# Keyteer/Mixed-precision_LU_Factorization

Hardware: AMD Instinct MI355X
Metric: LU GFLOP/s at N=32768 (1/2/4/8 GPUs); IR iterations to ||r||/||b||<1e-12 (higher is better)
Workload: dtype f64

## Files before the change

include/mpf_c.h:

```cpp
#ifndef MPF_C_H
#define MPF_C_H
#include <stdint.h>
#ifdef __cplusplus
extern "C" {
#endif

typedef struct mpf_ctx mpf_ctx;

enum { MPF_TRAIL_FP64 = 0, MPF_TRAIL_FP16 = 1, MPF_TRAIL_FP16X3 = 2 };

typedef struct mpf_opts {
    int32_t trailing;
    int32_t verbose;
    int32_t fused_panel;
    int32_t sync_timing;
    int32_t no_lookahead;
    int32_t superpanel;
    int32_t pivot_path;
    int32_t pivot_search;
} mpf_opts;

typedef struct mpf_stats {
    double ms_total;
    double ms_h2d, ms_d2h;
// ... 3 lines not shown
    int32_t hpanel_timeouts;
    int32_t info;
    int32_t gemm_launches;
    int32_t lookahead;
    int32_t superpanel;
    int32_t pivot_path;
    double gemm_flops;
    double gemm_bytes;
    double ms_gemm_big, gemm_big_flops, gemm_big_bytes;
    double ms_cvt;
    double ms_blockrow;
    int32_t gemm_big_launches;
    int32_t host_rows_streamed;
    int32_t host_late_segments;
    int32_t pivot_search;
} mpf_stats;

int mpf_create(mpf_ctx **out, int device);
int mpf_destroy(mpf_ctx *ctx);
int mpf_set_stream(mpf_ctx *ctx, void *hip_stream);
int mpf_synchronize(mpf_ctx *ctx);
const char *mpf_last_error(mpf_ctx *ctx);
int mpf_get_stats(mpf_ctx *ctx, mpf_stats *out);
int64_t mpf_hgetf2_capacity_rows(mpf_ctx *ctx, int32_t waiters, int32_t form);
int mpf_set_option(mpf_ctx *ctx, const char *name, int64_t value);
int mpf_get_option(mpf_ctx *ctx, const char *name, int64_t *value);
int mpf_option_name(int32_t index, char *buf, int64_t buflen);
int mpf_device_report(char *buf, int64_t buflen);


// ... 200 lines not shown
```

mixed-precision_lu_factorization_amd/__init__.py:

```python
import ctypes as C
import os
import subprocess

_HERE = os.path.dirname(os.path.abspath(__file__))
LIB_PATH = os.environ.get("MPF_LIB") or os.path.join(_HERE, "lib", "libmpf_amd.so")
PROBE_LIB_PATH = os.environ.get("MPF_PROBE_LIB") or os.path.join(_HERE, "lib", "libmpf_probe.so")

TRAIL_FP64 = 0
TRAIL_FP16 = 1
TRAIL_FP16X3 = 2

C_ABI_SYMBOLS = [
    "mpf_create", "mpf_destroy", "mpf_set_stream", "mpf_synchronize", "mpf_last_error", "mpf_get_stats",
    "mpf_device_report", "mpf_factor_host", "mpf_factor_dev", "mpf_double_to_fp16", "mpf_hdiv",
    "mpf_hgetf2_pivots", "mpf_hgetf2", "mpf_laswp", "mpf_dgetf2_npv", "mpf_dtrsm_llnu", "mpf_dgemm_minus",
    "mpf_solve_ir", "mpf_hgetf2_capacity_rows", "mpf_set_option", "mpf_get_option", "mpf_option_name", "mpf_hgemm_minus", "mpf_hgemm_minus_f32", "mpf_w32_from_f64", "mpf_w32_to_f64", "mpf_w32_laswp", "mpf_gesv", "mpf_matgen_dev", "mpf_matgen_cols_dev",
    "mpf_matgen_state", "mpf_rccl_unique_id", "mpf_rccl_init", "mpf_rccl_destroy", "mpf_rccl_version", "mpf_rccl_info", "mpf_rccl_bcast_probe", "mpf_factor_dist",
    "mpf_solve_ir_dist", "mpf_rccl_selftest", "mpf_check_plu_dev", "mpf_check_plu_host", "mpf_solve_ir_nrhs",
    "mpf_solve_gmres_ir", "mpf_trim", "mpf_dist_set_p2p",
    "mpf_solve_ir_trans", "mpf_lange", "mpf_geequ", "mpf_gecon", "mpf_gesvx",
    "mpf_getrs", "mpf_solve_ir_block", "mpf_gerfs", "mpf_gesvx_block",
    "mpf_dgetf2_piv", "mpf_solve_gmres_ir_block", "mpf_dgetf2_tp",
    "mpf_residual_x", "mpf_gerfsx",
]
# ... 3 lines not shown

class MpfOpts(C.Structure):
    _fields_ = [("trailing", C.c_int32), ("verbose", C.c_int32), ("fused_panel", C.c_int32),
                ("sync_timing", C.c_int32), ("no_lookahead", C.c_int32), ("superpanel", C.c_int32), ("pivot_path", C.c_int32), ("pivot_search", C.c_int32)]


class MpfStats(C.Structure):
    _fields_ = [("ms_total", C.c_double), ("ms_h2d", C.c_double), ("ms_d2h", C.c_double),
                ("ms_hpanel", C.c_double), ("ms_laswp", C.c_double), ("ms_dpanel", C.c_double),
                ("ms_trsm", C.c_double), ("ms_gemm", C.c_double), ("n", C.c_int64), ("nb", C.c_int32),
                ("panels", C.c_int32), ("hpanel_timeouts", C.c_int32), ("info", C.c_int32),
                ("gemm_launches", C.c_int32), ("lookahead", C.c_int32), ("superpanel", C.c_int32),
                ("pivot_path", C.c_int32), ("gemm_flops", C.c_double), ("gemm_bytes", C.c_double),
                ("ms_gemm_big", C.c_double), ("gemm_big_flops", C.c_double), ("gemm_big_bytes", C.c_double),
                ("ms_cvt", C.c_double), ("ms_blockrow", C.c_double), ("gemm_big_launches", C.c_int32), ("host_rows_streamed", C.c_int32),
                ("host_late_segments", C.c_int32), ("pivot_search", C.c_int32)]


class MpfIrStats(C.Structure):
    _fields_ = [("iterations", C.c_int32), ("converged", C.c_int32), ("rel_residual", C.c_double),
                ("history", C.c_double * 32), ("ms_total", C.c_double), ("stalled", C.c_int32), ("reserved", C.c_int32)]


class MpfGmresStats(C.Structure):
    _fields_ = [("outer_iterations", C.c_int32), ("inner_iterations", C.c_int32), ("converged", C.c_int32), ("budget_expired", C.c_int32),
                ("rel_residual", C.c_double), ("history", C.c_double * 32), ("ms_total", C.c_double)]


class MpfRcclInfo(C.Structure):
    _fields_ = [("version", C.c_int32), ("has_comm", C.c_int32), ("comm_count", C.c_int32), ("comm_rank", C.c_int32), ("has_p2p", C.c_int32),
                ("device", C.c_int32), ("visible_devices", C.c_int32), ("reserved", C.c_int32),
# ... 728 lines not shown
```

mixed-precision_lu_factorization_amd/csrc/laswp.hip:

```cpp
#include "mpf_internal.h"

constexpr int LASWP_CPB = 16;

__global__ __launch_bounds__(256) void laswp_plan_kernel(const int *ipiv, int k, int cols, MovedList *out) {
    __shared__ int slot[HP_MAXCOLS];
    __shared__ int rowof[2 * HP_MAXCOLS];
    __shared__ int content[2 * HP_MAXCOLS];
    __shared__ int used[2 * HP_MAXCOLS];
    __shared__ int count;
    const int t = threadIdx.x;
    for (int s = t; s < 2 * cols; s += 256) { content[s] = s; used[s] = s < cols; rowof[s] = s < cols ? k + s : -1; }
    if (t == 0) count = 0;
    __syncthreads();
    if (t < cols) {
        const int p = ipiv[t] - 1;
        int s;
        if (p < k + cols) s = p - k;
        else {
            int first = t;
            for (int i = 0; i < t; ++i)
                if (ipiv[i] - 1 == p) { first = i; break; }
            s = cols + first;
            if (first == t) { rowof[s] = p; used[s] = 1; }
        }
// ... 376 lines not shown
        const int64_t rows = N - r0;
        if (rows <= 0) continue;
        for (int b = p - sb; b < p; ++b) {
            if (world > 1 && b % world != rank) continue;
            const int w = nb;
            dim3 grid((unsigned)((rows + 255) / 256), (unsigned)((w + 15) / 16));
            double *Ab = A + (int64_t)(world > 1 ? b / world : b) * nb * lda;
            if (gather) lazy_gather_kernel<<<grid, 256, 0, c->stream>>>(Ab, lda, N, r0, w, Gmap, c->perm_tmp, rows);
            else lazy_scatter_kernel<<<grid, 256, 0, c->stream>>>(Ab, lda, N, r0, w, c->Fmap, c->perm_tmp, rows);
            lazy_copyback_kernel<<<grid, 256, 0, c->stream>>>(Ab, lda, N, r0, w, c->perm_tmp, rows);
        }
    }
    MPF_HIP_TRY(c, hipGetLastError());
    return 0;
}
```

mixed-precision_lu_factorization_amd/csrc/mpf_host.cpp:

```cpp
#include "solve_common.h"
#include "../../include/MPF.h"
#include <climits>
#include <cstdio>
#include <cstdlib>
#include <cstring>
#include <cmath>
#include <iostream>
#include <vector>
#include <mutex>
#include <functional>
#include <chrono>

static thread_local std::string g_noctx_err;

namespace {
struct OptDesc { const char *name, *env; size_t off; bool wide; long long lo, hi; };
#define OPT_I(field, env, lo, hi) {#field, env, offsetof(MpfTuning, field), false, lo, hi}
#define OPT_L(field, env, lo, hi) {#field, env, offsetof(MpfTuning, field), true, lo, hi}
const OptDesc kOpts[] = {
    OPT_I(safe_pivots, "MPF_SAFE_PIVOTS", 0, 1),
    OPT_I(pivot_fp64, "MPF_PIVOT_FP64", 0, 2),
    OPT_I(chain_pipeline, "MPF_CHAIN_PIPELINE", 0, 1),
    OPT_L(chain_pipeline_below, "MPF_CHAIN_PIPELINE_BELOW", 0, 1ll << 40),
    OPT_I(fp16_work32, "MPF_FP16_WORK32", 0, 1),
// ... 1 lines not shown
    OPT_I(superpanel_fp64, "MPF_SUPERPANEL_FP64", 1, 8),
    OPT_I(no_lookahead, "MPF_NO_LOOKAHEAD", 0, 1),
    OPT_I(verbose, "MPF_VERBOSE", 0, 1),
    OPT_I(timeline, "MPF_TIMELINE", 0, 1),
    OPT_L(hp_spin_limit, "MPF_HP_SPIN_LIMIT", 1, 1ll << 31),
    OPT_L(hp_gate_ticks, "MPF_HP_GATE_TICKS", 0, 1ll << 40),
    OPT_I(hp_acq_fence, "MPF_HP_ACQ_FENCE", 0, 1),
    OPT_I(hp_window, "MPF_HP_WINDOW", -1, 1 << 30),
    OPT_I(hgemm_pad, "MPF_HGEMM_PAD", 0, 65536),
    OPT_I(hgemm_split_pad, "MPF_HGEMM_SPLIT_PAD", 0, 65536),
    OPT_I(hgemm_big, "MPF_HGEMM_BIG", 0, 1),
    OPT_I(hgemm_big_tile, "MPF_HGEMM_BIG_TILE", 0, 5),
    OPT_I(hgemm_mfma16, "MPF_HGEMM_MFMA16", 0, 1),
    OPT_I(dgemm_dma, "MPF_DGEMM_DMA", 0, 1),
    OPT_I(lazy_gather, "MPF_LAZY_GATHER", 0, 1),
    OPT_I(dpanel_fused_form, "MPF_DPANEL_FUSED", 0, 1),
    OPT_I(dist_instalments, "MPF_DIST_INSTALMENTS", 0, 1),
    OPT_L(dist_instalment_min_bytes, "MPF_DIST_INSTALMENT_MIN_BYTES", 0, 1ll << 40),
    OPT_I(generic_fused, "MPF_GENERIC_FUSED", 0, 1),
    OPT_I(fp64_rowmajor, "MPF_FP64_ROWMAJOR", 0, 1),
    OPT_L(fp64_rowmajor_min_n, "MPF_FP64_ROWMAJOR_MIN_N", 0, 1ll << 40),
    OPT_I(trsm_laswp_fused, "MPF_TRSM_LASWP_FUSED", 0, 1),
    OPT_I(fp64_two_lanes, "MPF_FP64_TWO_LANES", 0, 1 << 30),
    OPT_I(fp64_lane_a_pct, "MPF_FP64_LANE_A_PCT", 20, 90),
    OPT_I(fp64_pair, "MPF_FP64_PAIR", 0, 1),
    OPT_L(fp64_pair_min_n, "MPF_FP64_PAIR_MIN_N", 0, 1ll << 40),
    OPT_I(event_timers, "MPF_EVENT_TIMERS", 0, 2),
    OPT_I(dist_world1_loop, "MPF_DIST_WORLD1_LOOP", 0, 1),
    OPT_I(gesv_fp64_tflops, "MPF_GESV_FP64_TFLOPS", 0, 1000),
    OPT_I(gate_wait_value, "MPF_GATE_WAIT_VALUE", 0, 1),
// ... 51 lines not shown
    if (e != hipSuccess || ndev == 0) return fail(nullptr, -3, "No HIP devices available.");
    if (device < 0 || device >= ndev) return fail(nullptr, -1, "mpf_create: bad device index");
    mpf_ctx *c = new mpf_ctx();
    tuning_from_env(c->tune);
    c->device = device;
    if (hipSetDevice(device) != hipSuccess) { delete c; return fail(nullptr, -2, "hipSetDevice failed"); }
    hipDeviceProp_t prop;
    if (hipGetDeviceProperties(&prop, device) == hipSuccess) c->num_cus = prop.multiProcessorCount;
    if (hipStreamCreateWithFlags(&c->stream, hipStreamNonBlocking) != hipSuccess) { delete c; return fail(nullptr, -2, "hipStreamCreate failed"); }
    c->own_stream = true;
    {
        int lo = 0, hi = 0;
        hipDeviceGetStreamPriorityRange(&lo, &hi);
        if (hipStreamCreateWithPriority(&c->pstream, hipStreamNonBlocking, hi) != hipSuccess) c->pstream = nullptr;
        if (hipStreamCreateWithPriority(&c->tstream, hipStreamNonBlocking, hi) != hipSuccess) c->tstream = nullptr;
    }
    if (hipMalloc((void **)&c->ws, sizeof(MpfWorkspace)) != hipSuccess) { hipStreamDestroy(c->stream); delete c; return fail(nullptr, -2, "hipMalloc(workspace) failed"); }
    hipMemset(c->ws, 0, sizeof(MpfWorkspace));
    if (hipExtMallocWithFlags((void **)&c->hp_signal, 8, hipMallocSignalMemory) != hipSuccess) { c->hp_signal = nullptr; (void)hipGetLastError(); }
    else hipMemset(c->hp_signal, 0, 8);
    hipEventCreate(&c->ev0);
    hipEventCreate(&c->ev1);
    *out = c;
    return 0;
}

int mpf_destroy(mpf_ctx *c) {
    if (!c) return 0;
    hipSetDevice(c->device);
    if (c->stream) hipStreamSynchronize(c->stream);
    if (c->ws) hipFree(c->ws);
    if (c->hp_signal) hipFree(c->hp_signal);
    mpf_rccl_destroy(c);
    sink_destroy(c);
    feed_destroy(c);
    if (c->ev0) hipEventDestroy(c->ev0);
    if (c->ev1) hipEventDestroy(c->ev1);
    if (c->pstream) { hipStreamSynchronize(c->pstream); hipStreamDestroy(c->pstream); }
    if (c->tstream) { hipStreamSynchronize(c->tstream); hipStreamDestroy(c->tstream); }
    if (c->xstream) { hipStreamSynchronize(c->xstream); hipStreamDestroy(c->xstream); }
    for (hipEvent_t e : c->ev_pool) hipEventDestroy(e);
    if (c->own_stream && c->stream) hipStreamDestroy(c->stream);
    delete c;
    return 0;
}

int mpf_set_stream(mpf_ctx *c, void *hip_stream) {
    if (!c) return -1;
    if (c->own_stream && c->stream) { hipStreamSynchronize(c->stream); hipStreamDestroy(c->stream); }
    c->stream = (hipStream_t)hip_stream;
    c->own_stream = false;
    return 0;
}

// ... 406 lines not shown
        StreamSwap sw(c, T);
        r.rc = ev.timed(f.st.ms_dpanel, T, [&] {
            int e = 0;
            for (int s = 0; s < np && !e; ++s) {
                e = launch_laswp_block_gated(c, f.d_A + nx * lda, lda, pc2, (int)nx + 32 * s, 32, f.d_ipiv + nx + 32 * s, N, 32 * (s + 1));
                if (!e) e = launch_dgetf2_npv_piece(c, Anx, lda, (int)(N - nx), pc2, f.o.fused_panel, (int)nx, s);
            }
            return e; });
        r.b = ev.get();
        hipEventRecord(r.b, T);
    }
    f.st.panels++;
    return r;
}

static int factor_epilogue(const FactorArgs &f, int rc, bool sink, int sb, bool side_streams) {
    mpf_ctx *c = f.c;
    hipStream_t S = c->stream;
    const int npanels = (int)((f.N + f.nb - 1) / f.nb);
    if (sink) sink_notify(c, npanels, S);
    else if (!rc) rc = f.ev.timed(f.st.ms_laswp, S, [&] { return launch_lazy_left_swaps(c, f.d_A, f.lda, f.N, f.nb, npanels, c->lists, sb); });
    hipError_t se = sink_stream_wait(c, S);
    hipError_t sp = side_streams ? sink_stream_wait(c, c->pstream) : hipSuccess;
    if (side_streams && c->tstream) { const hipError_t stt = sink_stream_wait(c, c->tstream); if (sp == hipSuccess) sp = stt; }
    if (!rc && (se != hipSuccess || sp != hipSuccess))
        return fail(c, -2, std::string("factorization failed: ") + hipGetErrorString(se != hipSuccess ? se : sp));
    f.ev.collect();
    f.st.lookahead = side_streams ? 1 : 0;
    return rc;
}

static int factor_lookahead(mpf_ctx *c, double *d_A, int64_t lda, int64_t N, int32_t nb, int32_t *d_ipiv,
                            const mpf_opts &o, mpf_stats &st) {
    hipStream_t S = c->stream, P = c->pstream;
    EvPool ev(c);
    ev.keep = &st.ms_gemm;
// ... 63 lines not shown
    return factor_epilogue(f, rc, sink, 1, true);
}

static bool pivots_fit_beside_update(const mpf_ctx *c, int64_t rows) {
    return c->num_cus <= 0 || (rows + HP_R - 1) / HP_R <= (int64_t)c->num_cus * 4 / 5;
}

static bool lane_split(const mpf_ctx *c, int64_t lo, int64_t hi, int64_t &cm) {
    const int64_t cw = hi - lo;
    if (cm >= 0 && (cm - lo) * 100 >= cw * (c->tune.fp64_lane_a_pct - 10)) return false;
    cm = lo + ((cw * c->tune.fp64_lane_a_pct / 100 + 127) / 128) * 128;
    if (cm > hi - 128) cm = hi - 128;
    return true;
}

struct PairHandover {
    int64_t k0 = 0;
    hipEvent_t chain = nullptr;
    hipEvent_t doneL = nullptr, doneR = nullptr;
    int64_t cm = -1;
};

static int factor_rm_pairs(mpf_ctx *c, EvPool &ev, mpf_stats &st, const mpf_opts &o, double *d_A, int64_t lda, int64_t N, int32_t nb,
                           int32_t *d_ipiv, hipEvent_t init_done, PairHandover &h) {
    hipStream_t S = c->stream, P = c->pstream, T = c->tstream;
    double *R = c->r64;
    const int64_t ldr = N, ldp = 2 * (int64_t)nb;
    const FactorArgs f{c, ev, st, o, d_A, lda, N, nb, d_ipiv};
    int rc = 0;
    hipEvent_t doneX = nullptr, doneA = nullptr, doneB = nullptr;
    int64_t cm = -1;
    int64_t k = h.k0;
    struct { bool valid = false; int64_t k = 0, c_lo = 0, w = 0; double *PI2 = nullptr; hipEvent_t ready = nullptr; } pendB;
    auto far_update = [&](int64_t kk, double *pi2, int64_t c_lo, int64_t w) -> int {
        const int64_t r0 = kk + 2 * (int64_t)nb;
        const int e = ev.timed(st.ms_gemm, S, [&] { return launch_dgemm_minus(c, w, N - r0, 2 * nb, R + kk * ldr + c_lo, ldr, pi2, ldp, R + r0 * ldr + c_lo, ldr); });
        count_gemm(st, o, N - r0, w, 2 * nb);
        return e;
    };
// ... 6 lines not shown
        hipEventRecord(doneB, S);
        pendB.valid = false;
        return e;
    };
    for (; rc == 0; k += 2 * (int64_t)nb) {
        const int64_t k1 = k + nb, k2 = k1 + nb, k3 = k2 + nb, k5 = k3 + 2 * (int64_t)nb;
        if (k5 + 256 > N || (N - k1) <= c->tune.fp64_pair_min_n) break;
        if (!pivots_fit_beside_update(c, N - k1)) break;
        const bool resplit = lane_split(c, k5, N, cm);
        double *Ak = d_A + k * lda + k, *Ak1 = d_A + k1 * lda + k1;
        double *PI = c->rm_pair + ((k / (2 * nb)) & 1) * N * ldp;
        double *PI2 = PI + (int64_t)nb * ldp;
        const MovedList *lk = c->lists + (k / nb), *lk1 = c->lists + (k1 / nb);
        hipEvent_t lt_ready = ev.get(), e1 = ev.get(), inner_done = ev.get(), chain1 = ev.get(), pi_ready = ev.get(), e2 = ev.get(),
                   chain2 = ev.get(), evX = ev.get(), evA = ev.get(), evB = ev.get(), ps1 = ev.get(), ps2 = ev.get();
        {
            if (doneB) hipStreamWaitEvent(P, doneB, 0);
            StreamSwap sw(c, P);
            rc = ev.timed(st.ms_cvt, P, [&] { return launch_transpose64(c, Ak + nb, lda, PI, ldp, N - k1, nb, true); });
            hipEventRecord(lt_ready, P);
        }
        if (rc) break;
        {
            hipStreamWaitEvent(T, h.chain, 0);
            hipStreamWaitEvent(T, doneX ? doneX : init_done, 0);
            StreamSwap sw(c, T);
            rc = ev.timed(st.ms_laswp, T, [&] { return launch_laswp_from_list_rm64(c, R + k1, ldr, k3 - k1, lk, (int64_t)LASWP_MAXMOVED * k1); });
            if (!rc) rc = ev.timed(st.ms_trsm, T, [&] { return launch_dtrsm_llnu_strided(c, nb, nb, Ak, lda, R + k * ldr + k1, ldr, 1); });
            hipStreamWaitEvent(T, lt_ready, 0);
            if (!rc) rc = ev.timed(st.ms_gemm, T, [&] { return launch_dgemm_minus(c, nb, N - k1, nb, R + k * ldr + k1, ldr, PI, ldp, R + k1 * ldr + k1, ldr); });
// ... 1 lines not shown
            if (!rc) rc = ev.timed(st.ms_cvt, T, [&] { return launch_transpose64(c, Ak1, lda, R + k1 * ldr + k1, ldr, N - k1, nb, false); });
            hipEventRecord(e1, T);
            if (!rc) rc = ev.timed(st.ms_trsm, T, [&] { return launch_dtrsm_llnu_strided(c, nb, nb, Ak, lda, R + k * ldr + k2, ldr, 1); });
            if (!rc) rc = ev.timed(st.ms_gemm, T, [&] { return launch_dgemm_minus(c, nb, N - k1, nb, R + k * ldr + k2, ldr, PI, ldp, R + k1 * ldr + k2, ldr); });
            count_gemm(st, o, N - k1, nb, nb);
            if (!rc) rc = ev.timed(st.ms_cvt, T, [&] { return launch_transpose64(c, d_A + k1 * lda + k, lda, R + k * ldr + k1, ldr, nb, k3 - k1, false); });
            hipEventRecord(inner_done, T);
        }
        if (rc) break;
        {
            hipStreamWaitEvent(P, e1, 0);
            if (doneA) hipStreamWaitEvent(P, doneA, 0);
            hipEventRecord(ps1, P);
            rc = panel_chain(f, k1, P);
            hipEventRecord(chain1, P);
            StreamSwap sw(c, P);
            hipStreamWaitEvent(P, inner_done, 0);
            if (!rc) rc = ev.timed(st.ms_laswp, P, [&] { return launch_laswp_from_list_rm64(c, PI - k1 * ldp, ldp, nb, lk1, 0); });
            if (!rc) rc = ev.timed(st.ms_cvt, P, [&] { return launch_transpose64(c, Ak1 + nb, lda, PI2 + nb, ldp, N - k2, nb, true); });
            hipEventRecord(pi_ready, P);
        }
        if (!rc) rc = flush_B(ps1);
        if (rc) break;
        {
            hipStreamWaitEvent(T, chain1, 0);
            StreamSwap sw(c, T);
            rc = ev.timed(st.ms_laswp, T, [&] { return launch_laswp_from_list_rm64(c, R + k2, ldr, nb, lk1, (int64_t)LASWP_MAXMOVED * k2); });
            if (!rc) rc = ev.timed(st.ms_trsm, T, [&] { return launch_dtrsm_llnu_strided(c, nb, nb, Ak1, lda, R + k1 * ldr + k2, ldr, 1); });
            hipStreamWaitEvent(T, pi_ready, 0);
            if (!rc) rc = ev.timed(st.ms_gemm, T, [&] { return launch_dgemm_minus(c, nb, N - k2, nb, R + k1 * ldr + k2, ldr, PI2 + nb, ldp, R + k2 * ldr + k2, ldr); });
// ... 45 lines not shown
        if (rc) break;
        doneA = ev.get();
        hipEventRecord(doneA, S);
        {
            if (doneB) hipStreamWaitEvent(T, doneB, 0);
            StreamSwap sw(c, T);
            rc = far_prep(cm, N - cm);
            hipEventRecord(evB, T);
        }
        if (rc) break;
        pendB.valid = true; pendB.k = k; pendB.PI2 = PI2; pendB.c_lo = cm; pendB.w = N - cm; pendB.ready = evB;
        h.chain = chain2;
        if (o.verbose) printf("panels k=%lld, %lld rows=%lld (row-major copy, paired: far update K = %d, lanes split at %lld)\n", (long long)k1, (long long)k2, (long long)(N - k1), 2 * nb, (long long)cm);
    }
    if (!rc) rc = flush_B(nullptr);
    h.k0 = k;
    h.doneL = doneA; h.doneR = doneB; h.cm = cm;
    return rc;
}

static int factor_lookahead_rm(mpf_ctx *c, double *d_A, int64_t lda, int64_t N, int32_t nb, int32_t *d_ipiv,
                               const mpf_opts &o, mpf_stats &st, bool pairs) {
    hipStream_t S = c->stream, P = c->pstream, T = c->tstream;
    EvPool ev(c);
    ev.keep = &st.ms_gemm;
    const FactorArgs f{c, ev, st, o, d_A, lda, N, nb, d_ipiv};
    int rc = 0;
    const bool sink = sink_take(c, d_A, lda, N, nb);
    double *R = c->r64;
    const int64_t ldr = N;
// ... 14 lines not shown
                if (!e) e = launch_dgetf2_npv(c, d_A, lda, (int)N, pc0, o.fused_panel, 0);
                return e; });
            hipEventRecord(e0, P);
        }
        st.panels++;
        if (!rc && pc0 < ce) rc = ev.timed(st.ms_cvt, S, [&] { return launch_transpose64(c, d_A + (int64_t)pc0 * lda, lda, R + pc0, ldr, N, ce - pc0, true); });
        hipStreamWaitEvent(S, e0, 0);
        chain_a = e0;
    }
    int64_t cm = -1;
    hipEvent_t doneL = nullptr, doneR = nullptr, prevR = nullptr;
    hipEvent_t init_done = ev.get();
    hipEventRecord(init_done, S);
    bool was_two = false;
    int64_t k0 = 0;
    if (pairs && !rc && !sink && !lp && T && N > 1) {
        PairHandover h;
        h.chain = chain_a;
        rc = factor_rm_pairs(c, ev, st, o, d_A, lda, N, nb, d_ipiv, init_done, h);
        if (h.k0 > 0) {
            k0 = h.k0; chain_a = h.chain; doneL = h.doneL; doneR = h.doneR; cm = h.cm;
            was_two = true;
        }
    }
    for (int64_t k = k0; k < N && rc == 0; k += nb) {
        const int pc = (int)((N - k) < nb ? (N - k) : nb);
        if (N - k <= 1 || k + pc >= N) break;
        const int64_t n = N - k - pc;
        const int64_t nx = k + pc;
        const int pc2 = (int)((N - nx) < nb ? (N - nx) : nb);
        const bool has_next = (N - nx) > 1;
        double *Ap = d_A + k * lda + k;
        double *LT = c->rm_lt + ((k / nb) & 1) * N * (int64_t)nb;
        const int64_t ns = has_next ? pc2 : n;
// ... 20 lines not shown
                if (sink && !rc && c_hi == N) sink_notify(c, (int)(kj / nb) + 1, S);
            }
            ++lseg;
            ce = lseg < lp->nseg ? lp->c0[lseg] : N;
            cm = -1;
            doneR = ev.get();
            hipEventRecord(doneR, S);
            doneL = nullptr;
        }
        if (rc) break;
        const int64_t cw = ce - nx - pc2;
        const bool want_two = T && c->tune.fp64_two_lanes > 0 && has_next && pivots_fit_beside_update(c, N - nx) &&
                              (N - nx) > c->tune.chain_pipeline_below && cw >= c->tune.fp64_two_lanes;
        if (!want_two) cm = -1;
        const bool resplit = want_two && lane_split(c, nx + pc2, ce, cm);
        if (cm >= 0) {
            const int64_t aw = cm - (nx + pc2);
            if (!was_two && k > 0) {
                doneL = ev.get();
                hipEventRecord(doneL, S);
            }
            hipEvent_t lt_ready = ev.get();
            {
                if (prevR) hipStreamWaitEvent(P, prevR, 0);
                StreamSwap sw(c, P);
                rc = ev.timed(st.ms_cvt, P, [&] { return launch_transpose64(c, Ap + pc, lda, LT, pc, n, pc, true); });
                hipEventRecord(lt_ready, P);
            }
            if (rc) break;
            hipEvent_t e1 = ev.get(), e2 = ev.get(), evA = ev.get(), evB = ev.get();
// ... 98 lines not shown
        }
        if (rc) break;
        if (cw > 0) {
            rc = ev.timed(st.ms_gemm, S, [&] { return launch_dgemm_minus(c, cw, n, pc, R + k * ldr + nx + pc2, ldr, LT, pc, R + nx * ldr + nx + pc2, ldr); });
            if (rc) break;
            count_gemm(st, o, n, cw, pc);
        }
        chain_a = next.a; chain_b = next.b;
        hipStreamWaitEvent(S, chain_a, 0);
        if (chain_b) hipStreamWaitEvent(S, chain_b, 0);
        if (o.verbose) printf("panel k=%lld rows=%lld cols=%d (look-ahead, row-major copy)\n", (long long)nx, (long long)(N - nx), pc2);
    }
    if (!rc && lp && lseg < lp->nseg) rc = fail(c, -1, "factor_lookahead_rm: a late column segment was never brought up to date (plan beyond the matrix)");
    if (T) stream_join(ev, T, S);
    stream_join(ev, P, S);
    return factor_epilogue(f, rc, sink, 1, true);
}

static int factor_superpanel(mpf_ctx *c, double *d_A, int64_t lda, int64_t N, int32_t nb, int32_t *d_ipiv, const mpf_opts &o,
                             mpf_stats &st, int sb, bool overlap) {
    hipStream_t S = c->stream, P = overlap ? c->pstream : c->stream;
    hipStream_t Ci = (overlap && c->tstream) ? c->tstream : c->stream;
    const bool lanes = Ci != S;
    EvPool ev(c);
    ev.keep = &st.ms_gemm;
    const FactorArgs f{c, ev, st, o, d_A, lda, N, nb, d_ipiv};
    int rc = 0;
    const bool split = o.trailing == MPF_TRAIL_FP16X3;
    const bool f64 = o.trailing == MPF_TRAIL_FP64;
    const bool use32 = !f64 && c->tune.fp16_work32 != 0 && N > (int64_t)(sb + 1) * nb;
    float *W = nullptr;
// ... 219 lines not shown
    if (o.trailing != MPF_TRAIL_FP64) {
        const int64_t kimg = (int64_t)sb * nb < 8 * HP_MAXCOLS ? (int64_t)sb * nb : 8 * HP_MAXCOLS;
        int e = mpf_ensure_h_images(c, N + HP_MAXCOLS + 64, (int)kimg, sb > 1); if (e) return e;
    }
    { const int e = mpf_factor_setup(c, N, nb, (int)((N + nb - 1) / nb), !generic); if (e) return e; }
    if (piv64) { const int e = piv64 == 2 ? dgetf2_tp_reserve(c, (int)N) : dgetf2_piv_reserve(c, (int)N); if (e) return e; }
    mpf_stats st{};
    st.n = N; st.nb = nb; st.superpanel = sb;
    st.pivot_search = piv64;
    const bool lookahead = !o.sync_timing && !o.no_lookahead && !c->tune.no_lookahead && c->pstream != nullptr;
    const bool use_rm = !generic && sb <= 1 && lookahead && o.trailing == MPF_TRAIL_FP64 && c->tune.fp64_rowmajor &&
                        N >= c->tune.fp64_rowmajor_min_n && N > nb && mpf_ensure_rowmajor_copy(c, N, N, nb) == 0;
    bool use_pairs = use_rm && c->tune.fp64_pair && c->tune.fp64_two_lanes > 0 && c->tstream && nb % 16 == 0 && N > c->tune.fp64_pair_min_n;
    if (use_pairs && !pivots_fit_beside_update(c, N - nb)) use_pairs = false;
    if (use_pairs && c->rm_pair.grow(4 * N * (int64_t)nb) != hipSuccess) { (void)hipGetLastError(); use_pairs = false; }
    if (c->late && !use_rm) {
        const int e = feed_finish(c);
        c->late = nullptr;
        if (e) return e;
    }
    MPF_HIP_TRY(c, hipEventRecord(c->ev0, c->stream));
    int rc;
    if (generic) rc = factor_generic(c, d_A, lda, N, nb, d_ipiv, o, st, force_generic, piv64);
    else if (sb > 1) rc = factor_superpanel(c, d_A, lda, N, nb, d_ipiv, o, st, sb, lookahead);
    else if (use_rm) rc = factor_lookahead_rm(c, d_A, lda, N, nb, d_ipiv, o, st, use_pairs);
    else if (lookahead) rc = factor_lookahead(c, d_A, lda, N, nb, d_ipiv, o, st);
    else {
        mpf_opts o2 = o;
        rc = factor_sync_timed(c, d_A, lda, N, nb, d_ipiv, o2, st);
    }
// ... 21 lines not shown

static int ensure_host_copies(mpf_ctx *c, int64_t N) {
    MPF_HIP_TRY(c, c->host_A.grow(N * N));
    MPF_HIP_TRY(c, c->host_P.grow(N));
    return 0;
}

int mpf_trim(mpf_ctx *c) {
    if (!c) return -1;
    MPF_HIP_TRY(c, hipSetDevice(c->device));
    MPF_HIP_TRY(c, hipStreamSynchronize(c->stream));
    c->host_A.release(); c->host_P.release(); c->host_A0.release();
    sink_trim(c);
    feed_trim(c);
    c->r64.release(); c->rm_tmp.release(); c->rm_lt.release(); c->rm_pair.release();
    c->w32.release();
    return 0;
}

int mpf_factor_host(mpf_ctx *c, double *A_host, int64_t N, int32_t nb, int32_t *ipiv_host, const mpf_opts *opts) {
    if (!c || !A_host || !ipiv_host) return -1;
    if (N <= 0 || nb <= 0) return fail(c, -1, "mpf_factor: N and panel width must be positive");
    MPF_HIP_TRY(c, hipSetDevice(c->device));
    { const int e = ensure_host_copies(c, N); if (e) return e; }
    double *dA = c->host_A;
    int32_t *dP = c->host_P;
    const size_t bytes = (size_t)N * (size_t)N * sizeof(double), pbytes = (size_t)N * sizeof(int32_t);
    const bool want_sink = c->tune.host_sink && N >= c->tune.host_sink_min_n && c->pstream != nullptr && !(opts && (opts->sync_timing || opts->no_lookahead)) &&
                           !(opts && opts->trailing != MPF_TRAIL_FP64) && !(opts && opts->pivot_path == 1) &&
                           !(opts && opts->pivot_search != 0) && !c->tune.pivot_fp64;
// ... 247 lines not shown
```

mixed-precision_lu_factorization_amd/csrc/mpf_internal.h:

```cpp
#pragma once
#include <hip/hip_runtime.h>
#include <stdint.h>
#include <string>
#include <vector>
#include <functional>
#include "../../include/mpf_c.h"

constexpr int HP_R = 256;
constexpr int HP_T = 512;
constexpr int HP_MAXG = 256;
constexpr int HP_MAXCOLS = 256;
constexpr int LASWP_MAXMOVED = 2 * HP_MAXCOLS;

struct MovedList {
    int n;
    int pad[3];
    int src[LASWP_MAXMOVED];
    int dst[LASWP_MAXMOVED];
};

struct MpfWorkspace {
    unsigned long long cand[2][HP_MAXG];
    int flags[16];
    unsigned long long rowbuf[2][HP_MAXG][HP_MAXCOLS / 2];
// ... 18 lines not shown
    int superpanel_fp64 = 1;
    int no_lookahead = 0;
    int verbose = 0;
    int timeline = 0;
    long long hp_spin_limit = 1ll << 21;
    long long hp_gate_ticks = 200000000ll;
    int hp_window = -1;
    int hp_acq_fence = 0;
    int hgemm_pad = 0;
    int hgemm_split_pad = 32768;
    int hgemm_big = 1;
    int hgemm_mfma16 = 1;
    int hgemm_big_tile = 0;
    int dgemm_dma = 1;
    int lazy_gather = 1;
    int dpanel_fused_form = 1;
    int dist_instalments = 1;
    long long dist_instalment_min_bytes = 8ll << 20;
    int generic_fused = 1;
    int fp64_rowmajor = 1;
    long long fp64_rowmajor_min_n = 8192;
    int trsm_laswp_fused = 1;
    int fp64_two_lanes = 8192;
    int dist_solve_p2p = 0;
    int host_sink = 1;
    int hp_local_xcd = 1;
    int hp_half_slabs = 1;
    int hp_half_slabs_rows = 16384;
    int sink_trace = 0;
    int host_late_parts = 3;
// ... 45 lines not shown
    int64_t cap() const { return cap_; }
private:
    T *p_ = nullptr;
    int64_t cap_ = 0;
};

struct mpf_ctx {
    MpfTuning tune;
    unsigned attr_done = 0;
    unsigned attr_big = 0;
    int device = 0;
    hipStream_t stream = nullptr;
    bool own_stream = false;
    hipStream_t pstream = nullptr;
    hipStream_t tstream = nullptr;
    hipStream_t xstream = nullptr;
    std::vector<hipEvent_t> ev_pool;
    MpfWorkspace *ws = nullptr;
    hipEvent_t ev0 = nullptr, ev1 = nullptr;
    std::string err;
    mpf_stats stats{};
    int num_cus = 0;
    Buf<double> solve_buf;
    int64_t solve_n = 0;
    Buf<unsigned short> h_L, h_U;
    int64_t h_rows = 0;
    Buf<unsigned short> h_Lb[2];
    int h_kmax = 0;
    unsigned hp_seq = 0;
    unsigned long long *hp_signal = nullptr;
    Buf<int32_t> perm_buf;
    Buf<MovedList> lists;
    Buf<int> Fmap;
    Buf<double> perm_tmp;
    Buf<double> trsv_inv;
    Buf<double> trsv_inv256;
    Buf<int> trsv_cnt;
    Buf<double> krylov;
    Buf<double> res_part;
    Buf<double> ext_part, ext_red, ext_vec;
    Buf<double> blk_tiles, blk_part;
    Buf<int> blk_mask;
    Buf<double> blk_red;
    Buf<int> blk_colarg;
    Buf<double> gm_part, gm_out, gm_ctl;
    Buf<double> dtiles;
    Buf<float> w32;
    Buf<double> r64;
    bool hgemm_standalone = false;
// ... 52 lines not shown
constexpr int HP_FP64_WINDOW_ROWS = 20000;
int hp_query_residency(mpf_ctx *c);
int launch_hgetf2_gate(mpf_ctx *c, int target);
int launch_laswp_block(mpf_ctx *c, double *A, int64_t lda, int64_t ncols, int k, int cols, const int *d_ipiv, int64_t nrows);
int launch_laswp_block_gated(mpf_ctx *c, double *A, int64_t lda, int64_t ncols, int k, int cols, const int *d_ipiv, int64_t nrows, int target);
int dgetf2_npv_pieces(mpf_ctx *c, int cols);
int launch_dgetf2_npv_piece(mpf_ctx *c, double *P, int64_t ld, int rows, int cols, int fused, int info_base, int piece);
int launch_dpanel_tile_copy(mpf_ctx *c, double *dst, int64_t ld, int piece);
int launch_hgetf2_generic(mpf_ctx *c, const double *A64, int64_t lda, uint16_t *P16, int64_t ld16, int rows, int cols,
                          int ipiv_offset, int *d_ipiv, uint16_t *out16, int64_t ldo);
int launch_laswp_seq(mpf_ctx *c, double *A, int64_t lda, int64_t ncols, int k, int cols, const int *d_ipiv, int64_t nrows);
int launch_laswp_from_list(mpf_ctx *c, double *A, int64_t lda, int64_t ncols, const MovedList *ml);
int launch_laswp_from_list_hole(mpf_ctx *c, double *A, int64_t lda, int64_t ncols, const MovedList *ml, int64_t hole_from, int64_t hole_len);
int launch_lazy_left_swaps(mpf_ctx *c, double *A, int64_t lda, int64_t N, int nb, int npanels, const MovedList *lists, int sb = 1,
                           int world = 1, int rank = 0);
struct LatePlan {
    int nseg = 0;
    int64_t c0[4] = {0, 0, 0, 0};
    int q[4] = {0, 0, 0, 0};
    unsigned *flags = nullptr;
    unsigned seq = 0;
    double *snapshot = nullptr;
    bool taken = false;
    bool snapped[4] = {false, false, false, false};
};
int launch_late_wait(mpf_ctx *c, const unsigned *flag, unsigned seq);
int feed_start(mpf_ctx *c, const double *A_host, double *d_A, int64_t N, LatePlan *lp);
int feed_finish(mpf_ctx *c);
void feed_destroy(mpf_ctx *c);
void feed_trim(mpf_ctx *c);
// ... 166 lines not shown
```

Baseline: 53700.

## Apply deferred left-side row swaps in bands on a low-priority side stream

Adds a left-bands mode, on by default, that records a per-panel row map and composes the maps into source indices. It then writes the finished L columns straight from the row-major copy into their final pivoted positions, running on a new low-priority stream while the factorization continues. This replaces the end-of-factorization lazy left-swap pass with incremental band moves that overlap the trailing updates. In exchange it allocates two N×(N/nb) int map buffers, which is large at N=32768, and it adds transposes and stream contention that can compete with the main GEMM work.

Result: no change. 54100 (median of 6 runs) (+0.7%).

```diff
diff --git a/include/mpf_c.h b/include/mpf_c.h
--- a/include/mpf_c.h
+++ b/include/mpf_c.h
@@ -41,6 +41,7 @@
     int32_t host_rows_streamed;
     int32_t host_late_segments;
     int32_t pivot_search;
+    int32_t left_bands;
 } mpf_stats;
 
 int mpf_create(mpf_ctx **out, int device);
diff --git a/mixed-precision_lu_factorization_amd/__init__.py b/mixed-precision_lu_factorization_amd/__init__.py
--- a/mixed-precision_lu_factorization_amd/__init__.py
+++ b/mixed-precision_lu_factorization_amd/__init__.py
@@ -41,7 +41,7 @@
                 ("pivot_path", C.c_int32), ("gemm_flops", C.c_double), ("gemm_bytes", C.c_double),
                 ("ms_gemm_big", C.c_double), ("gemm_big_flops", C.c_double), ("gemm_big_bytes", C.c_double),
                 ("ms_cvt", C.c_double), ("ms_blockrow", C.c_double), ("gemm_big_launches", C.c_int32), ("host_rows_streamed", C.c_int32),
-                ("host_late_segments", C.c_int32), ("pivot_search", C.c_int32)]
+                ("host_late_segments", C.c_int32), ("pivot_search", C.c_int32), ("left_bands", C.c_int32)]
 
 
 class MpfIrStats(C.Structure):
diff --git a/mixed-precision_lu_factorization_amd/csrc/laswp.hip b/mixed-precision_lu_factorization_amd/csrc/laswp.hip
--- a/mixed-precision_lu_factorization_amd/csrc/laswp.hip
+++ b/mixed-precision_lu_factorization_amd/csrc/laswp.hip
@@ -414,3 +414,96 @@
     MPF_HIP_TRY(c, hipGetLastError());
     return 0;
 }
+
+__global__ __launch_bounds__(256) void left_band_panel_map_kernel(int *__restrict__ M, long long n, long long r_lo, const MovedList *__restrict__ ml) {
+    __shared__ int m[256];
+    const long long r0 = r_lo + (long long)blockIdx.x * 256;
+    const int t = threadIdx.x;
+    m[t] = (int)(r0 + t);
+    __syncthreads();
+    int cnt = ml->n;
+    if (cnt > LASWP_MAXMOVED) cnt = LASWP_MAXMOVED;
+    for (int i = t; i < cnt; i += 256) {
+        const long long d = ml->dst[i], s = ml->src[i];
+        if (d >= r0 && d < r0 + 256 && s >= r_lo && s < n) m[d - r0] = (int)s;
+    }
+    __syncthreads();
+    if (r0 + t < n) M[r0 + t] = m[t];
+}
+__global__ __launch_bounds__(256) void left_band_src_kernel(const int *__restrict__ maps, long long n, int nb, long long d0, long long d1,
+                                                           int *__restrict__ src) {
+    const long long d = d0 + (long long)blockIdx.x * 256 + threadIdx.x;
+    if (d >= d1) return;
+    long long s = d;
+    for (int q = (int)(d / nb); q >= 1; --q) {
+        const long long v = maps[(long long)q * n + s];
+        if (v >= (long long)q * nb && v < n) s = v;
+        src[(long long)(q - 1) * n + d] = (int)s;
+    }
+}
+constexpr int LB_ROWS = 32;
+template <bool VEC>
+__global__ __launch_bounds__(256) void left_band_move_kernel(double *__restrict__ A, long long lda, const double *__restrict__ R, long long n,
+                                                            int nb, long long d0, long long d1, const int *__restrict__ src) {
+    __shared__ double t[LB_ROWS][66];
+    const long long r0 = d0 + (long long)blockIdx.x * LB_ROWS, c0 = (long long)blockIdx.y * 64;
+    const long long rl = (r0 + LB_ROWS < d1 ? r0 + LB_ROWS : d1) - 1;
+    if (c0 >= (rl / nb) * nb) return;
+    if (VEC) {
+        const int cx = (threadIdx.x & 31) * 2, ry = threadIdx.x >> 5;
+        const long long col = c0 + cx;
+        const long long b = col / nb;
+#pragma unroll
+        for (int i = 0; i < LB_ROWS / 8; ++i) {
+            const int rr = ry + 8 * i;
+            const long long d = r0 + rr;
+            if (d < d1 && col < (d / nb) * nb) {
+                const long long s = src[b * n + d];
+                const double2 v = *(const double2 *)(R + s * n + col);
+                t[rr][cx] = v.x; t[rr][cx + 1] = v.y;
+            }
+        }
+    } else {
+        const int cx = threadIdx.x & 63, ry = threadIdx.x >> 6;
+        const long long col = c0 + cx;
+        const long long b = col / nb;
+#pragma unroll
+        for (int i = 0; i < LB_ROWS / 4; ++i) {
+            const int rr = ry + 4 * i;
+            const long long d = r0 + rr;
+            if (d < d1 && col < (d / nb) * nb) t[rr][cx] = R[(long long)src[b * n + d] * n + col];
+        }
+    }
+    __syncthreads();
+    const int tx = threadIdx.x & (LB_ROWS - 1), ty = threadIdx.x / LB_ROWS;
+    const long long d = r0 + tx;
+    if (d >= d1) return;
+    const long long owed = (d / nb) * nb;
+#pragma unroll
+    for (int i = 0; i < 64 / (256 / LB_ROWS); ++i) {
+        const int cc = ty + (256 / LB_ROWS) * i;
+        if (c0 + cc < owed) A[d + (c0 + cc) * lda] = t[tx][cc];
+    }
+}
+int launch_left_band_map(mpf_ctx *c, int p, int64_t N, int nb, const MovedList *ml) {
+    const int64_t r_lo = (int64_t)p * nb;
+    if (p < 1 || r_lo >= N) return 0;
+    if (c->band_maps.cap() < ((int64_t)p + 1) * N) { c->err = "left bands: map store too small"; return -1; }
+    left_band_panel_map_kernel<<<(unsigned)((N - r_lo + 255) / 256), 256, 0, c->stream>>>(c->band_maps + (int64_t)p * N, N, r_lo, ml);
+    MPF_HIP_TRY(c, hipGetLastError());
+    return 0;
+}
+int launch_left_band(mpf_ctx *c, double *A, int64_t lda, const double *R, int64_t N, int nb, int64_t d0, int64_t d1) {
+    if (d0 < nb) d0 = nb;
+    if (d1 > N) d1 = N;
+    if (d1 <= d0) return 0;
+    const int64_t pl = (d1 - 1) / nb;
+    if (c->band_maps.cap() < (pl + 1) * N || c->band_src.cap() < pl * N) { c->err = "left bands: map store too small"; return -1; }
+    left_band_src_kernel<<<(unsigned)((d1 - d0 + 255) / 256), 256, 0, c->stream>>>(c->band_maps, N, nb, d0, d1, c->band_src);
+    dim3 grid((unsigned)((d1 - d0 + LB_ROWS - 1) / LB_ROWS), (unsigned)((pl * nb + 63) / 64));
+    if (grid.y > 65535) { c->err = "left bands: too many columns"; return -1; }
+    if (((N | nb) & 1) == 0) left_band_move_kernel<true><<<grid, 256, 0, c->stream>>>(A, lda, R, N, nb, d0, d1, c->band_src);
+    else left_band_move_kernel<false><<<grid, 256, 0, c->stream>>>(A, lda, R, N, nb, d0, d1, c->band_src);
+    MPF_HIP_TRY(c, hipGetLastError());
+    return 0;
+}
diff --git a/mixed-precision_lu_factorization_amd/csrc/mpf_host.cpp b/mixed-precision_lu_factorization_amd/csrc/mpf_host.cpp
--- a/mixed-precision_lu_factorization_amd/csrc/mpf_host.cpp
+++ b/mixed-precision_lu_factorization_amd/csrc/mpf_host.cpp
@@ -39,6 +39,7 @@
     OPT_I(hgemm_mfma16, "MPF_HGEMM_MFMA16", 0, 1),
     OPT_I(dgemm_dma, "MPF_DGEMM_DMA", 0, 1),
     OPT_I(lazy_gather, "MPF_LAZY_GATHER", 0, 1),
+    OPT_I(left_bands, "MPF_LEFT_BANDS", 0, 2),
     OPT_I(dpanel_fused_form, "MPF_DPANEL_FUSED", 0, 1),
     OPT_I(dist_instalments, "MPF_DIST_INSTALMENTS", 0, 1),
     OPT_L(dist_instalment_min_bytes, "MPF_DIST_INSTALMENT_MIN_BYTES", 0, 1ll << 40),
@@ -120,6 +121,7 @@
         hipDeviceGetStreamPriorityRange(&lo, &hi);
         if (hipStreamCreateWithPriority(&c->pstream, hipStreamNonBlocking, hi) != hipSuccess) c->pstream = nullptr;
         if (hipStreamCreateWithPriority(&c->tstream, hipStreamNonBlocking, hi) != hipSuccess) c->tstream = nullptr;
+        if (hipStreamCreateWithPriority(&c->bstream, hipStreamNonBlocking, lo) != hipSuccess) c->bstream = nullptr;
     }
     if (hipMalloc((void **)&c->ws, sizeof(MpfWorkspace)) != hipSuccess) { hipStreamDestroy(c->stream); delete c; return fail(nullptr, -2, "hipMalloc(workspace) failed"); }
     hipMemset(c->ws, 0, sizeof(MpfWorkspace));
@@ -144,6 +146,7 @@
     if (c->ev1) hipEventDestroy(c->ev1);
     if (c->pstream) { hipStreamSynchronize(c->pstream); hipStreamDestroy(c->pstream); }
     if (c->tstream) { hipStreamSynchronize(c->tstream); hipStreamDestroy(c->tstream); }
+    if (c->bstream) { hipStreamSynchronize(c->bstream); hipStreamDestroy(c->bstream); }
     if (c->xstream) { hipStreamSynchronize(c->xstream); hipStreamDestroy(c->xstream); }
     for (hipEvent_t e : c->ev_pool) hipEventDestroy(e);
     if (c->own_stream && c->stream) hipStreamDestroy(c->stream);
@@ -580,12 +583,12 @@
     return r;
 }
 
-static int factor_epilogue(const FactorArgs &f, int rc, bool sink, int sb, bool side_streams) {
+static int factor_epilogue(const FactorArgs &f, int rc, bool sink, int sb, bool side_streams, bool left_done = false) {
     mpf_ctx *c = f.c;
     hipStream_t S = c->stream;
     const int npanels = (int)((f.N + f.nb - 1) / f.nb);
     if (sink) sink_notify(c, npanels, S);
-    else if (!rc) rc = f.ev.timed(f.st.ms_laswp, S, [&] { return launch_lazy_left_swaps(c, f.d_A, f.lda, f.N, f.nb, npanels, c->lists, sb); });
+    else if (!rc && !left_done) rc = f.ev.timed(f.st.ms_laswp, S, [&] { return launch_lazy_left_swaps(c, f.d_A, f.lda, f.N, f.nb, npanels, c->lists, sb); });
     hipError_t se = sink_stream_wait(c, S);
     hipError_t sp = side_streams ? sink_stream_wait(c, c->pstream) : hipSuccess;
     if (side_streams && c->tstream) { const hipError_t stt = sink_stream_wait(c, c->tstream); if (sp == hipSuccess) sp = stt; }
@@ -679,6 +682,49 @@
     return true;
 }
 
+struct LeftBands {
+    const FactorArgs &f;
+    double *R;
+    int mode;
+    int64_t next = 0, done;
+    int rc = 0;
+    LeftBands(const FactorArgs &f_, double *R_, int mode_) : f(f_), R(R_), mode(mode_), done(f_.nb) {}
+    void step(int64_t k, hipEvent_t a, hipEvent_t b, bool bulk) {
+        if (!mode || rc || k != next || k >= f.N) return;
+        mpf_ctx *c = f.c;
+        hipStream_t B = c->bstream;
+        const int64_t N = f.N;
+        const int nb = f.nb, pc = (int)((N - k) < nb ? (N - k) : nb);
+        const int64_t n = N - k - pc;
+        if (a) hipStreamWaitEvent(B, a, 0);
+        if (b) hipStreamWaitEvent(B, b, 0);
+        StreamSwap sw(c, B);
+        if (n > 0) rc = f.ev.timed(f.st.ms_cvt, B, [&] { return launch_transpose64(c, f.d_A + k * f.lda + k + pc, f.lda, R + (k + pc) * N + k, N, n, pc, true); });
+        if (!rc && k > 0) rc = f.ev.timed(f.st.ms_laswp, B, [&] {
+            int e = launch_left_band_map(c, (int)(k / nb), N, nb, c->lists + (k / nb));
+            if (!e && (mode == 1 || bulk)) e = band(k + pc);
+            return e; });
+        next = k + pc;
+    }
+    int band(int64_t upto) {
+        if (upto <= done) return 0;
+        const int e = launch_left_band(f.c, f.d_A, f.lda, R, f.N, f.nb, done, upto);
+        done = upto;
+        f.st.left_bands++;
+        return e;
+    }
+    int finish(int rc_sched, hipEvent_t a, hipEvent_t b) {
+        if (!mode) return rc_sched;
+        mpf_ctx *c = f.c;
+        if (!rc_sched) {
+            while (!rc && next < f.N) step(next, a, b, false);
+            if (!rc) { StreamSwap sw(c, c->bstream); rc = f.ev.timed(f.st.ms_laswp, c->bstream, [&] { return band(f.N); }); }
+        }
+        stream_join(f.ev, c->bstream, c->stream);
+        return rc_sched ? rc_sched : rc;
+    }
+};
+
 struct PairHandover {
     int64_t k0 = 0;
     hipEvent_t chain = nullptr;
@@ -687,7 +733,7 @@
 };
 
 static int factor_rm_pairs(mpf_ctx *c, EvPool &ev, mpf_stats &st, const mpf_opts &o, double *d_A, int64_t lda, int64_t N, int32_t nb,
-                           int32_t *d_ipiv, hipEvent_t init_done, PairHandover &h) {
+                           int32_t *d_ipiv, hipEvent_t init_done, PairHandover &h, LeftBands &lb) {
     hipStream_t S = c->stream, P = c->pstream, T = c->tstream;
     double *R = c->r64;
     const int64_t ldr = N, ldp = 2 * (int64_t)nb;
@@ -724,6 +770,7 @@
         const MovedList *lk = c->lists + (k / nb), *lk1 = c->lists + (k1 / nb);
         hipEvent_t lt_ready = ev.get(), e1 = ev.get(), inner_done = ev.get(), chain1 = ev.get(), pi_ready = ev.get(), e2 = ev.get(),
                    chain2 = ev.get(), evX = ev.get(), evA = ev.get(), evB = ev.get(), ps1 = ev.get(), ps2 = ev.get();
+        lb.step(k, h.chain, nullptr, true);
         {
             if (doneB) hipStreamWaitEvent(P, doneB, 0);
             StreamSwap sw(c, P);
@@ -755,6 +802,7 @@
             hipEventRecord(ps1, P);
             rc = panel_chain(f, k1, P);
             hipEventRecord(chain1, P);
+            lb.step(k1, chain1, nullptr, true);
             StreamSwap sw(c, P);
             hipStreamWaitEvent(P, inner_done, 0);
             if (!rc) rc = ev.timed(st.ms_laswp, P, [&] { return launch_laswp_from_list_rm64(c, PI - k1 * ldp, ldp, nb, lk1, 0); });
@@ -830,6 +878,7 @@
         if (o.verbose) printf("panels k=%lld, %lld rows=%lld (row-major copy, paired: far update K = %d, lanes split at %lld)\n", (long long)k1, (long long)k2, (long long)(N - k1), 2 * nb, (long long)cm);
     }
     if (!rc) rc = flush_B(nullptr);
+    if (!rc) rc = lb.rc;
     h.k0 = k;
     h.doneL = doneA; h.doneR = doneB; h.cm = cm;
     return rc;
@@ -874,10 +923,13 @@
     hipEventRecord(init_done, S);
     bool was_two = false;
     int64_t k0 = 0;
+    const int64_t npan = (N + nb - 1) / nb;
+    const bool bands = c->tune.left_bands && !sink && !lp && c->bstream && N > nb && c->band_maps.cap() >= npan * N && c->band_src.cap() >= npan * N;
+    LeftBands lb(f, R, bands ? c->tune.left_bands : 0);
     if (pairs && !rc && !sink && !lp && T && N > 1) {
         PairHandover h;
         h.chain = chain_a;
-        rc = factor_rm_pairs(c, ev, st, o, d_A, lda, N, nb, d_ipiv, init_done, h);
+        rc = factor_rm_pairs(c, ev, st, o, d_A, lda, N, nb, d_ipiv, init_done, h, lb);
         if (h.k0 > 0) {
             k0 = h.k0; chain_a = h.chain; doneL = h.doneL; doneR = h.doneR; cm = h.cm;
             was_two = true;
@@ -928,6 +980,8 @@
                               (N - nx) > c->tune.chain_pipeline_below && cw >= c->tune.fp64_two_lanes;
         if (!want_two) cm = -1;
         const bool resplit = want_two && lane_split(c, nx + pc2, ce, cm);
+        lb.step(k, chain_a, chain_b, cm >= 0);
+        if (lb.rc) { rc = lb.rc; break; }
         if (cm >= 0) {
             const int64_t aw = cm - (nx + pc2);
             if (!was_two && k > 0) {
@@ -1056,7 +1110,8 @@
     if (!rc && lp && lseg < lp->nseg) rc = fail(c, -1, "factor_lookahead_rm: a late column segment was never brought up to date (plan beyond the matrix)");
     if (T) stream_join(ev, T, S);
     stream_join(ev, P, S);
-    return factor_epilogue(f, rc, sink, 1, true);
+    rc = lb.finish(rc, chain_a, chain_b);
+    return factor_epilogue(f, rc, sink, 1, true, lb.mode != 0);
 }
 
 static int factor_superpanel(mpf_ctx *c, double *d_A, int64_t lda, int64_t N, int32_t nb, int32_t *d_ipiv, const mpf_opts &o,
@@ -1306,6 +1361,10 @@
     bool use_pairs = use_rm && c->tune.fp64_pair && c->tune.fp64_two_lanes > 0 && c->tstream && nb % 16 == 0 && N > c->tune.fp64_pair_min_n;
     if (use_pairs && !pivots_fit_beside_update(c, N - nb)) use_pairs = false;
     if (use_pairs && c->rm_pair.grow(4 * N * (int64_t)nb) != hipSuccess) { (void)hipGetLastError(); use_pairs = false; }
+    if (use_rm && c->tune.left_bands) {
+        const int64_t need = ((N + nb - 1) / nb) * N;
+        if (c->band_maps.grow(need) != hipSuccess || c->band_src.grow(need) != hipSuccess) { (void)hipGetLastError(); c->band_maps.release(); c->band_src.release(); }
+    }
     if (c->late && !use_rm) {
         const int e = feed_finish(c);
         c->late = nullptr;
@@ -1357,6 +1416,7 @@
     sink_trim(c);
     feed_trim(c);
     c->r64.release(); c->rm_tmp.release(); c->rm_lt.release(); c->rm_pair.release();
+    c->band_maps.release(); c->band_src.release();
     c->w32.release();
     return 0;
 }
diff --git a/mixed-precision_lu_factorization_amd/csrc/mpf_internal.h b/mixed-precision_lu_factorization_amd/csrc/mpf_internal.h
--- a/mixed-precision_lu_factorization_amd/csrc/mpf_internal.h
+++ b/mixed-precision_lu_factorization_amd/csrc/mpf_internal.h
@@ -56,6 +56,7 @@
     int hgemm_big_tile = 0;
     int dgemm_dma = 1;
     int lazy_gather = 1;
+    int left_bands = 1;
     int dpanel_fused_form = 1;
     int dist_instalments = 1;
     long long dist_instalment_min_bytes = 8ll << 20;
@@ -131,6 +132,7 @@
     bool own_stream = false;
     hipStream_t pstream = nullptr;
     hipStream_t tstream = nullptr;
+    hipStream_t bstream = nullptr;
     hipStream_t xstream = nullptr;
     std::vector<hipEvent_t> ev_pool;
     MpfWorkspace *ws = nullptr;
@@ -150,6 +152,7 @@
     Buf<MovedList> lists;
     Buf<int> Fmap;
     Buf<double> perm_tmp;
+    Buf<int> band_maps, band_src;
     Buf<double> trsv_inv;
     Buf<double> trsv_inv256;
     Buf<int> trsv_cnt;
@@ -232,6 +235,8 @@
 int launch_laswp_from_list_hole(mpf_ctx *c, double *A, int64_t lda, int64_t ncols, const MovedList *ml, int64_t hole_from, int64_t hole_len);
 int launch_lazy_left_swaps(mpf_ctx *c, double *A, int64_t lda, int64_t N, int nb, int npanels, const MovedList *lists, int sb = 1,
                            int world = 1, int rank = 0);
+int launch_left_band_map(mpf_ctx *c, int p, int64_t N, int nb, const MovedList *ml);
+int launch_left_band(mpf_ctx *c, double *A, int64_t lda, const double *R, int64_t N, int nb, int64_t d0, int64_t d1);
 struct LatePlan {
     int nseg = 0;
     int64_t c0[4] = {0, 0, 0, 0};
```
